# jeffchy/RE2NN-SEQ

Measured on AMD Instinct MI355X. Metric: tagged tokens/sec @ batch=256, seqlen=64; achieved HBM GB/s vs peak, higher is better.
Workload: dtype f32; 1 GPU; ATIS-BIO-sized onehot i-FST (--method onehot --independent 2): V=950 S=71 C=128, batch 256 x seqlen 64 per GPU, lengths U[5,64]; batches_rotated=4, parallelism=batch-sharded x1 (weights replicated)

## Files before the change

### re2nn-seq_amd/csrc/chain_regs.hip

```cpp
#include <hip/hip_runtime.h>
#include <hip/hip_ext.h>

#include "common.hip.h"
#include "host_util.hip.h"
#include "chain_regs.hip.h"

namespace farnn {

int launch_chain_regs(const RegsParams &p, bool maxsr, bool score, hipStream_t s, hipEvent_t e0, hipEvent_t e1) {
    const int NP = RG_NWC * p.G;
    const bool dest = p.dest && !maxsr;
    const size_t lds = (size_t)regs_lds(p.L, p.SP, NP, p.sp.c16, p.sp.Kc, score, RG_RQ, score && bs_label_map_path(p.sp), dest).total * sizeof(float);
    const dim3 grid(2 * p.B), block(RG_WAVES * 64);
    int rc;
    const bool nlx = p.nl != FARNN_NL_NONE && p.nl != FARNN_NL_RELU;
    const bool lmo = score && bs_label_map_path(p.sp);
#define FARNN_LAUNCH_REGS5(MX, SC, NX, LM, DS)                                                 \
    do {                                                                                       \
        if ((rc = raise_lds_limit(chain_regs_kernel<MX, SC, NX, LM, DS>, lds))) return rc;     \
        if (e0 && e1)                                                                          \
            hipExtLaunchKernelGGL((chain_regs_kernel<MX, SC, NX, LM, DS>), grid, block, (uint32_t)lds, s, e0, e1, 0, p); \
        else                                                                                   \
            chain_regs_kernel<MX, SC, NX, LM, DS><<<grid, block, lds, s>>>(p);                \
    } while (0)
#if defined(FARNN_AB)
#define FARNN_LAUNCH_REGS4(MX, SC, NX, LM) do { if (!MX && dest) FARNN_LAUNCH_REGS5(MX, SC, NX, LM, !MX); else FARNN_LAUNCH_REGS5(MX, SC, NX, LM, false); } while (0)
#else
#define FARNN_LAUNCH_REGS4(MX, SC, NX, LM)                                                     \
    do {                                                                                       \
        if (!MX && dest) FARNN_LAUNCH_REGS5(MX, SC, NX, LM, !MX);                              \
        else if constexpr (MX) FARNN_LAUNCH_REGS5(MX, SC, NX, LM, false);                      \
        else return fail(FARNN_EINVAL, "FARNN_NODEST=1: the source-split compute wavefronts of the sum semiring are compiled into the A/B " \
                                       "build only (FARNN_LIB=.../libfarnn_hip_probes.so, csrc/build.py --probes)%s%s"); \
    } while (0)
#endif
#define FARNN_LAUNCH_REGS3(MX, SC, NX) do { if (SC && lmo) FARNN_LAUNCH_REGS4(MX, SC, NX, SC); else FARNN_LAUNCH_REGS4(MX, SC, NX, false); } while (0)
#define FARNN_LAUNCH_REGS(MX, SC) do { if (nlx) FARNN_LAUNCH_REGS3(MX, SC, true); else FARNN_LAUNCH_REGS3(MX, SC, false); } while (0)
    if (maxsr) { if (score) FARNN_LAUNCH_REGS(true, true); else FARNN_LAUNCH_REGS(true, false); }
    else       { if (score) FARNN_LAUNCH_REGS(false, true); else FARNN_LAUNCH_REGS(false, false); }
#undef FARNN_LAUNCH_REGS
#undef FARNN_LAUNCH_REGS3
#undef FARNN_LAUNCH_REGS4
#undef FARNN_LAUNCH_REGS5
    FARNN_HIP_TRY(hipGetLastError());
    return FARNN_OK;
}

}

#if defined(FARNN_PROBES)
extern "C" int farnn_debug_wg_stamps(long long *out, int n_workgroups) {
    if (!out || n_workgroups < 0 || n_workgroups > farnn::WG_STAMP_MAX) return FARNN_EINVAL;
    if (hipDeviceSynchronize() != hipSuccess) return FARNN_EIO;
    return hipMemcpyFromSymbol(out, HIP_SYMBOL(farnn::g_wg_stamps), sizeof(long long) * 16 * (size_t)n_workgroups) == hipSuccess ? FARNN_OK : FARNN_EIO;
}
#endif
```

### re2nn-seq_amd/csrc/chain_regs.hip.h

```cpp
#pragma once
#include "common.hip.h"
#include "score_params.hip.h"
#include "launch_order.hip.h"
#include "chain_regs_params.hip.h"
#include "beside.hip.h"

#ifndef FARNN_ABLATE
#define FARNN_ABLATE 0
#endif

namespace farnn {

__device__ __forceinline__ void lds_flag_set(int *f, int v) {
    asm volatile("" ::: "memory");
    __hip_atomic_store(f, v, __ATOMIC_RELAXED, __HIP_MEMORY_SCOPE_WORKGROUP);
}
__device__ __forceinline__ int lds_flag_get(const int *f) {
    const int v = __hip_atomic_load(f, __ATOMIC_RELAXED, __HIP_MEMORY_SCOPE_WORKGROUP);
    asm volatile("" ::: "memory");
    return v;
}
template <int PSTR = RG_PART_STRIDE>
__device__ __forceinline__ int regs_flag_newest(const float *fbase, int lane) {
    const int *f = reinterpret_cast<const int *>(fbase) + 4 * (lane < RG_NWC ? lane : 0);
    const int v0 = lds_flag_get(f), v1 = lds_flag_get(f + PSTR);
    return max(v0, v1);
}
template <int PSTR = RG_PART_STRIDE>
__device__ __forceinline__ bool regs_rows_reached(const float *fbase, int lane, int rows) {
    return __ballot(regs_flag_newest<PSTR>(fbase, lane) < rows + 1) == 0ull;
}
template <int PSTR = RG_PART_STRIDE>
__device__ __forceinline__ int regs_rows_done(const float *fbase, int lane) {
    int v = regs_flag_newest<PSTR>(fbase, lane);
#pragma unroll
    for (int off = 1; off < 8; off <<= 1) v = min(v, __shfl_xor(v, off, WAVE));
    return __builtin_amdgcn_readfirstlane(v) - 1;
}

__device__ __forceinline__ float quad_sum(float x) {
    x += __int_as_float(__builtin_amdgcn_update_dpp(0, __float_as_int(x), 0xB1, 0xf, 0xf, true));
    x += __int_as_float(__builtin_amdgcn_update_dpp(0, __float_as_int(x), 0x4E, 0xf, 0xf, true));
    return x;
}
__device__ __forceinline__ float quad_max(float x) {
    x = fmaxf(x, __int_as_float(__builtin_amdgcn_update_dpp(0, __float_as_int(x), 0xB1, 0xf, 0xf, true)));
    x = fmaxf(x, __int_as_float(__builtin_amdgcn_update_dpp(0, __float_as_int(x), 0x4E, 0xf, 0xf, true)));
    return x;
}

}
#include "chain_wide.hip.h"
#include "chain_dest.hip.h"
namespace farnn {

#if defined(FARNN_PROBES)
constexpr int WG_STAMP_MAX = 4096;
__device__ long long g_wg_stamps[16 * WG_STAMP_MAX];
#define FARNN_RG_STAMP(i) do { if (probe && lane == 0) stamps[i] = (long long)__builtin_amdgcn_s_memtime(); } while (0)
#else
#define FARNN_RG_STAMP(i) do { } while (0)
#endif

template <bool MAXSR, bool SCORE, bool NLX, int RQ = RG_RQ, int D = RG_D, bool LMO = false, bool DEST = false>
__device__ __forceinline__ void chain_regs_body(const RegsParams &p, float *smem, const int tid, const int item, int *b_out) {
    constexpr bool WIDE = RQ != RG_RQ;
    static_assert(!DEST || (!WIDE && !MAXSR), "the destination-split form exists for the narrow kernel and the sum semiring");
    constexpr int PSTR = WIDE ? rgw_part_stride(RQ) : RG_PART_STRIDE;
    constexpr int NG = WIDE ? RGW_NG : RG_NG;
    const int lane = tid & 63;
    const int w = __builtin_amdgcn_readfirstlane(tid >> 6);
    constexpr int nthreads = RG_WAVES * 64;
    const int dir = item & 1, slot = item >> 1;
    const int S = p.S, SP = p.SP, G = p.G, RPG = p.RPG, NP = RG_NWC * G;
    const int PS = WIDE ? p.PS : SP;
    const bool lm_path = SCORE && (LMO || bs_label_map_path(p.sp));
    const RegsLds lds = regs_lds(p.L, SP, NP, p.sp.c16, p.sp.Kc, SCORE, RQ, lm_path, DEST);
    long long *tokoff = reinterpret_cast<long long *>(smem + lds.tok);
    float *part = smem + lds.part, *ol = smem + lds.ol, *hist = smem + lds.hist;
    float *ab = smem + lds.ab, *scl = smem + lds.scl, *obuf = smem + lds.obuf;
    int *misc = reinterpret_cast<int *>(smem + lds.misc);

    int b = p.order ? p.order[slot] : slot;
    int len_sel = -1;
    if (p.sort) b = select_by_length_rank(p.len, p.B, p.L, p.pair ? folded_rank(slot, p.B) : slot, reinterpret_cast<int *>(hist), tid, nthreads, &len_sel);
    if (b_out) *b_out = b;
    const int len = len_sel >= 0 ? len_sel : clamp_len(p.len[b], p.L);
    const int nsteps = p.full ? p.L : len;
    const float *hinit = dir == 0 ? p.h0 : p.hT;
#if defined(FARNN_PROBES)
    __shared__ long long stamps[8];
    const bool quiet = (p.dbg & 2048) != 0;
    const bool probe = ((p.dbg & 32768) && nsteps == p.L && p.L >= 32) || quiet;
    if (w == 0) FARNN_RG_STAMP(0);
#endif

    constexpr bool PRIME_EARLY = DEST && (!SCORE || LMO);
    DestRing<RD_D, RD_LPR> dring;
    if constexpr (PRIME_EARLY)
        if (w < RG_NWC && nsteps > 0) regs_dest_prime<RD_D, RD_LPR>(p, dir, w, lane, nsteps, len, b, dring);
    for (int k = tid; k < nsteps; k += nthreads) {
        const int idx = (dir == 0) ? k : (k < len ? len - 1 - k : k);
        tokoff[k] = (long long)clamp_tok(p.x[(long long)b * p.L + idx], p.V) * p.blk * 4;
    }
    for (int j = tid; j < SP; j += nthreads) ol[j] = (p.o && j < S) ? p.o[j] : 1.0f;
    for (int j = tid; j < (nsteps + 1) * SP; j += nthreads) hist[j] = (j < S) ? hinit[j] : 0.0f;
    if (tid < 32) misc[tid] = tid == RGM_ACQ ? -1 : 0;
    if (tid < 2) part[tid * PSTR + PSTR - 1] = MAXSR ? -INFINITY : 0.0f;
    if (tid < 2 * 4 * RG_NWC) {
        const int fb = tid / (4 * RG_NWC), fk = tid % (4 * RG_NWC);
// ... 16 lines not shown
    int kmid = 0, pubmax = 0;
    if (SCORE) bs_halves(dir, len, nsteps, kmid, pubmax);
    BesideParams bs;
    bs.A = p.A; bs.Bk = p.Bk; bs.B = p.B; bs.L = p.L; bs.SP = p.SP; bs.CPR = p.CPR; bs.prog = p.prog; bs.arr = p.arr;
    bs.done = p.done; bs.spin = p.spin; bs.dbg = p.dbg; bs.sp = p.sp;
    bs.epoch = (SCORE && w >= RG_NWC) ? (p.done ? bs_launch_epoch(p.done, lane) : p.epoch_host) : 0u;
    int wr_next = 0;
    unsigned lm_pk0 = 0u, lm_pk1 = 0u;
    if (lm_path) lm_load_packed(bs.sp.lm, lane, lm_pk0, lm_pk1);
    if (w < RG_NWC) {
        if constexpr (WIDE) {
            if (nsteps > 0) {
                __builtin_amdgcn_s_setprio(2);
                regs_compute_wide<MAXSR, NLX, RQ, D>(p, dir, w, lane, nsteps, tokoff, part, ol, hist, smem + lds.xch);
                __builtin_amdgcn_s_setprio(0);
                if (w == 0) FARNN_RG_STAMP(2);
#if defined(FARNN_PROBES)
                if (!SCORE && probe && !quiet && w == 0 && lane == 0)
                    printf("seq %d dir %d (wide): setup %lld, chain %lld (%lld per step)\n", b, dir, stamps[1] - stamps[0], stamps[2] - stamps[1],
                           (stamps[2] - stamps[1]) / nsteps);
#endif
            }
        } else if constexpr (DEST) {
            if (nsteps > 0) {
                __builtin_amdgcn_s_setprio(2);
#if defined(FARNN_PROBES)
                const bool probe_ = probe;
#else
                const bool probe_ = false;
#endif
                if constexpr (!PRIME_EARLY) regs_dest_prime<RD_D, RD_LPR>(p, dir, w, lane, nsteps, len, b, dring);
                regs_compute_dest<NLX, RD_D, RD_LPR>(p, dir, w, lane, nsteps, tokoff, part + NP * PS, ol, hist, smem + lds.xd, probe_, b, dring);
                __builtin_amdgcn_s_setprio(0);
                if (w == 0) FARNN_RG_STAMP(2);
#if defined(FARNN_PROBES)
                if (!SCORE && probe && !quiet && w == 0 && lane == 0)
                    printf("seq %d dir %d (destination split): setup %lld, chain %lld (%lld per step)\n", b, dir, stamps[1] - stamps[0], stamps[2] - stamps[1],
                           (stamps[2] - stamps[1]) / nsteps);
#endif
            }
        } else if (nsteps > 0) {
            __builtin_amdgcn_s_setprio(2);
            int g = lane / p.CPR;
            const int c = lane - g * p.CPR;
            const bool active = g < G;
            if (!active) g = 0;
            const int gid = w * G + g, row0 = gid * RPG;
            unsigned voff[RG_RQ];
#pragma unroll
            for (int u = 0; u < RG_RQ; u++) voff[u] = ((unsigned)(row0 + u) * (unsigned)SP + (unsigned)c * 4u) * 4u;
            const char *Mbase = reinterpret_cast<const char *>(dir == 0 ? p.Mf : p.Mb);
            const int rows_w = G * RPG;
            const int rj = lane >> 2, rs = lane & 3;
            const int my_row = w * rows_w + rj;
            const bool my_valid = rj < rows_w && my_row < S;
            const bool my_writer = my_valid && rs == 0;
            const float my_o = my_valid ? ol[my_row] : 1.0f;
            const float c_pre = dir == 0 ? my_o : 1.0f, c_post = dir == 0 ? 1.0f : my_o;
            const float ninf = -INFINITY;
            bool okrow[RG_RQ];
#pragma unroll
            for (int u = 0; u < RG_RQ; u++) okrow[u] = u < RPG && row0 + u < S;
            constexpr int NQI = (RG_NWC * RG_MAXG + 3) / 4;
            const float *ident = part + RG_PART_STRIDE - 1;
            float *dump = part + 2 * RG_PART_STRIDE;
            const float *qptr[NQI];
// ... 163 lines not shown
                    }
#endif
                    FARNN_RG_PHASE(3);
                }
            }
            if (lane == 0) lds_flag_set(reinterpret_cast<int *>(fslot), nsteps + 1);
#if defined(FARNN_PROBES)
            if (probe && w == 0 && lane == 0 && (p.dbg & 256))
                printf("seq %d dir %d chain phases, cycles per step: block wait %lld, fma + store + issue %lld, partner wait + partial reads %lld, reduce + exchange %lld\n",
                       b, dir, ph[0] / nsteps, ph[1] / nsteps, ph[2] / nsteps, ph[3] / nsteps);
#endif
#undef FARNN_RG_PHASE
#undef FARNN_RG_ISSUE
#undef FARNN_RG_BASE
#undef FARNN_RG_WINDOW
#undef FARNN_RG_WAIT
            __builtin_amdgcn_s_setprio(0);
            if (w == 0) FARNN_RG_STAMP(2);
#if defined(FARNN_PROBES)
            if (!SCORE && probe && !quiet && w == 0 && lane == 0)
                printf("seq %d dir %d: setup %lld, chain %lld (%lld per step)\n", b, dir, stamps[1] - stamps[0], stamps[2] - stamps[1],
                       (stamps[2] - stamps[1]) / nsteps);
#endif
        }
    } else if (w == RG_NWC) {
        if (SCORE && dir == 0) {
            for (int i = nsteps + lane; i < p.L; i += WAVE)
                if (p.sp.tags) p.sp.tags[(long long)b * p.L + i] = -1;
            if (p.sp.scores)
                for (long long e = (long long)nsteps * p.sp.K + lane; e < (long long)p.L * p.sp.K; e += WAVE)
                    p.sp.scores[(long long)b * p.L * p.sp.K + e] = 0.0f;
        }
        int published = -1;
        auto copy_rows = [&](int r0, int r1) {
            const float *src = hist + r0 * SP;
            float *dst = stash + (long long)r0 * SP;
            const int nfl = (r1 - r0 + 1) * SP;
            if (SCORE) {
                for (int j = 2 * lane; j < nfl; j += 2 * WAVE) st2_agent(dst + j, src[j], src[j + 1]);
            } else {
                for (int j = lane; j < nfl; j += WAVE) dst[j] = src[j];
            }
        };
        if (!SCORE && !p.A) wr_next = nsteps + 1;
        while (wr_next <= nsteps) {
            const int done = nsteps > 0 ? regs_rows_done<PSTR>(sflag, lane) : 0;
            if (done < wr_next) { __builtin_amdgcn_s_sleep(1); continue; }
            if (SCORE && nsteps > 0 && wr_next > pubmax && done >= nsteps) break;
            const int hi = min(done, (SCORE && wr_next <= pubmax) ? pubmax : nsteps);
            copy_rows(wr_next, hi);
            wr_next = hi + 1;
            if (SCORE && hi < nsteps && published < pubmax) {
                published = hi;
                asm volatile("s_waitcnt vmcnt(0)" ::: "memory");
                if (lane == 0)
                    __hip_atomic_store(p.prog + (long long)dir * p.B + b, ((unsigned long long)bs.epoch << 32) | (unsigned)published,
                                       __ATOMIC_RELAXED, __HIP_MEMORY_SCOPE_AGENT);
            }
        }
    } else if (SCORE) {
        const int fo = bs_flat_offset(bs, b, lane);
        if (lane == 0) misc[RGM_FOFF] = fo;
        const long long foff = fo;
        unsigned mine = 0u;
        int acq = -1;
        const unsigned long long *oprog = p.prog + (long long)(dir ^ 1) * p.B + b;
        const int kfirst = dir == 0 ? kmid : kmid - 1, kstep = dir == 0 ? 1 : -1, klast = dir == 0 ? ntl : -1;
        if constexpr (!LMO)
        for (int k = kfirst; k != klast && !lm_path; k += kstep) {
            int na, nb;
            bs_tile_need(k, len, nsteps, na, nb);
            const int need_own = dir == 0 ? na : nb, need_oth = dir == 0 ? nb : na;
            if (nsteps - need_own < p.solo_margin) break;
            while (!regs_rows_reached<PSTR>(sflag, lane, need_own)) __builtin_amdgcn_s_sleep(4);
            if (need_oth > acq) {
                int pr = -1;
                for (;;) {
                    pr = lane == 0 ? bs_read_prog(oprog, bs.epoch) : 0;
                    pr = __builtin_amdgcn_readfirstlane(pr);
                    if (pr >= need_oth) break;
                    if (regs_rows_reached<PSTR>(sflag, lane, nsteps)) break;
                    __builtin_amdgcn_s_sleep(8);
                }
                if (pr < need_oth) break;
                __builtin_amdgcn_fence(__ATOMIC_ACQUIRE, "agent");
                acq = pr;
            }
            {
                const rg_f32x4 none[NG] = {};
                bs_score_tiles<false, RG_WAVES, NG, RG_NWC>(bs, b, dir, len, nsteps, k, -1, hist, nullptr, nullptr, ab, scl, foff, 0, lane, none);
            }
            mine |= 1u << k;
        }
        {
            int slot = 0;
            for (int k = kfirst; k != klast && slot < RG_NOB; k += kstep) {
                if ((mine >> k) & 1u) continue;
                int na, nb;
                bs_tile_need(k, len, nsteps, na, nb);
                const int need_oth = dir == 0 ? nb : na;
                if (need_oth > acq) {
                    int pr = -1;
                    for (;;) {
                        pr = lane == 0 ? bs_read_prog(oprog, bs.epoch) : 0;
                        pr = __builtin_amdgcn_readfirstlane(pr);
                        if (pr >= need_oth) break;
                        if (regs_rows_reached<PSTR>(sflag, lane, nsteps)) break;
                        __builtin_amdgcn_s_sleep(16);
                    }
                    if (pr < need_oth) break;
                    __builtin_amdgcn_fence(__ATOMIC_ACQUIRE, "agent");
                    acq = pr;
                }
                bs_park_rows<NG, (LMO && WIDE) ? NG / 2 : NG>(bs, b, dir, len, nsteps, k, obuf + slot * RG_TT * SP, lane);
                if (lane == 0) misc[RGM_PARK + slot] = k + 1;
                slot++;
            }
        }
        if (lane == 0) { misc[RGM_MINE] = (int)mine; misc[RGM_ACQ] = acq; }
        FARNN_RG_STAMP(3);
    }
    if constexpr (!SCORE) {
        if (b_out && dir == 0 && w == RG_WAVES - 1) {
            int partsum = 0;
            if (p.sp.flat && !p.sp.offs)
                for (int j = lane; j < b; j += WAVE) partsum += clamp_len(p.len[j], p.L);
#pragma unroll
            for (int off = 32; off >= 1; off >>= 1) partsum += __shfl_xor(partsum, off, WAVE);
            if (lane == 0) { misc[RGM_FOFF] = partsum; misc[RGM_FOFF + 1] = len; }
        }
        return;
    }

    if (w == 0) FARNN_RG_STAMP(4);
    bs_finish<RG_WAVES, NG, RG_WAVES - 1, RG_NWC, true, LMO>(bs, b, dir, len, nsteps, kmid, hist, ab, scl, obuf, misc, w, lane, lm_pk0, lm_pk1, bs.epoch,
        [&]() {
            if (w == RG_NWC)
                for (; wr_next <= nsteps; wr_next++)
                    for (int j = 2 * lane; j < SP; j += 2 * WAVE)
                        st2_agent(stash + (long long)wr_next * SP + j, hist[wr_next * SP + j], hist[wr_next * SP + j + 1]);
        },
        [&]() {
            if (w == RG_NWC) {
                asm volatile("s_waitcnt vmcnt(0)" ::: "memory");
                if (lane == 0)
                    __hip_atomic_store(p.prog + (long long)dir * p.B + b, ((unsigned long long)bs.epoch << 32) | (unsigned)nsteps,
                                       __ATOMIC_RELAXED, __HIP_MEMORY_SCOPE_AGENT);
            }
        });
#if defined(FARNN_PROBES)
    if (quiet && tid == 0 && item < WG_STAMP_MAX) {
        long long *o = g_wg_stamps + 16 * (long long)item + 8;
        o[0] = stamps[1] - stamps[0]; o[1] = stamps[2] - stamps[1]; o[2] = stamps[3] - stamps[2]; o[3] = stamps[4] - stamps[2];
        o[4] = (long long)__builtin_amdgcn_s_memtime() - stamps[4];
    }
    if (probe && !quiet && tid == 0) {
        const long long e = (long long)__builtin_amdgcn_s_memtime();
        printf("seq %d dir %d: setup %lld, chain %lld (%lld per step), scorer alone until +%lld, all waves at the meeting point +%lld, "
               "tiles + arrival %lld; tiles alone %d of %d\n", b, dir, stamps[1] - stamps[0], stamps[2] - stamps[1],
               (stamps[2] - stamps[1]) / nsteps, stamps[3] - stamps[2], stamps[4] - stamps[2], e - stamps[4],
               __popc((unsigned)misc[RGM_MINE]), ntl);
    }
#endif
}

template <bool MAXSR, bool SCORE, bool NLX, bool LMO = false, bool DEST = false>
__global__ void __launch_bounds__(RG_WAVES * 64, 4)
chain_regs_kernel(const RegsParams p) {
    extern __shared__ __align__(16) float smem[];
#if defined(FARNN_PROBES)
    long long w0r = 0, w0c = 0;
    if ((p.dbg & 2048) && threadIdx.x == 0) { w0r = (long long)__builtin_amdgcn_s_memrealtime(); w0c = (long long)__builtin_amdgcn_s_memtime(); }
    int b_probe = -1;
    chain_regs_body<MAXSR, SCORE, NLX, RG_RQ, RG_D, LMO, DEST>(p, smem, (int)threadIdx.x, (int)blockIdx.x, &b_probe);
    if ((p.dbg & 2048) && threadIdx.x == 0 && blockIdx.x < WG_STAMP_MAX) {
        const long long w1r = (long long)__builtin_amdgcn_s_memrealtime(), w1c = (long long)__builtin_amdgcn_s_memtime();
        unsigned hwid, xcc;
        asm volatile("s_getreg_b32 %0, hwreg(HW_REG_HW_ID)" : "=s"(hwid));
        asm volatile("s_getreg_b32 %0, hwreg(HW_REG_XCC_ID)" : "=s"(xcc));
        long long *o = g_wg_stamps + 16 * (long long)blockIdx.x;
        o[0] = b_probe; o[1] = b_probe >= 0 ? (long long)p.len[b_probe] : -1; o[2] = w0r; o[3] = w1r; o[4] = w1c - w0c;
        o[5] = xcc & 15u; o[6] = (hwid >> 13) & 7u; o[7] = (hwid >> 8) & 15u;
    }
#else
    chain_regs_body<MAXSR, SCORE, NLX, RG_RQ, RG_D, LMO, DEST>(p, smem, (int)threadIdx.x, (int)blockIdx.x, nullptr);
#endif
}

template <bool MAXSR, bool SCORE, bool NLX, int RQ, int D>
__global__ void __launch_bounds__(RG_WAVES * 64, 2)
chain_wide_kernel(const RegsParams p) {
    extern __shared__ __align__(16) float smem[];
    chain_regs_body<MAXSR, SCORE, NLX, RQ, D>(p, smem, (int)threadIdx.x, (int)blockIdx.x, nullptr);
}

template <bool MAXSR, bool NLX, int RQ>
__global__ void __launch_bounds__(RG_WAVES * 64, 4)
chain_wide_paired_kernel(const RegsParams p) {
    extern __shared__ __align__(16) float smem[];
    chain_regs_body<MAXSR, true, NLX, RQ, 2, true>(p, smem, (int)threadIdx.x, (int)blockIdx.x, nullptr);
}

}
```

### re2nn-seq_amd/csrc/chain_regs_params.hip.h

```cpp
#pragma once
#include <hip/hip_runtime.h>
#include "common.hip.h"
#include "score_params.hip.h"

namespace farnn {

constexpr int RG_NWC = 6;
constexpr int RG_WAVES = 8;
constexpr int RG_D = 4;
constexpr int RG_RQ = 4;
constexpr int RG_MAXG = 4;
constexpr int RG_MAXSP = 72;
constexpr int RG_PART_STRIDE = RG_NWC * RG_MAXG * RG_MAXSP;
constexpr int RGW_G = 2;
constexpr int RGW_NP = RG_NWC * RGW_G;
constexpr int RGW_MAXSP = 128;
constexpr int RGW_MAXRQ = 11;
__host__ __device__ constexpr int rgw_part_stride(int rq) { return rq <= 9 ? 1536 : 2048; }
constexpr int RGW_XCH = 32;
constexpr int RD_LPR = 5;
constexpr int RD_XS = 80;
constexpr int RD_D = 4;
constexpr int RD_XD_FLOATS = 2 * RD_XS + 128;

// ... 28 lines not shown
    int G, RPG, NP, CPR, SP, rows;
    bool ok;
    bool wide;
    int RQ, D, PS;
};

inline RegsGeom regs_geometry(int S) {
    RegsGeom g;
    g.wide = false; g.RQ = RG_RQ; g.D = RG_D; g.PS = 0;
    g.SP = round_up(S, 4);
    g.CPR = g.SP / 4;
    g.ok = g.CPR <= 64 && S >= 1;
    g.G = g.ok ? 64 / g.CPR : 1;
    if (g.G > RG_MAXG) g.G = RG_MAXG;
    g.NP = RG_NWC * g.G;
    g.RPG = (S + g.NP - 1) / g.NP;
    if (g.RPG > RG_RQ) g.ok = false;
    g.rows = (g.NP - 1) * g.RPG + RG_RQ;
    if (g.NP * g.SP + 4 * RG_NWC + 4 * (64 - g.G * g.CPR) >= RG_PART_STRIDE) g.ok = false;
    if (!g.ok && S > 4 * RG_RQ && g.SP <= RGW_MAXSP) {
        g.wide = true;
        g.G = RGW_G; g.NP = RGW_NP;
        g.RPG = (S + g.NP - 1) / g.NP;
        g.RQ = g.RPG <= 8 ? 8 : (g.RPG <= 9 ? 9 : RGW_MAXRQ);
        g.D = 4;
        g.rows = g.NP * g.RPG;
        g.PS = ((g.SP + 15) & ~31) + 16;
        g.ok = g.RPG <= RGW_MAXRQ && g.NP * g.PS + 4 * RG_NWC + 4 * (64 - g.G * g.CPR) < rgw_part_stride(g.RQ);
    }
    return g;
}

struct RegsLds {
    int tok, hp, part, ol, hist, ab, scl, obuf, misc, xch, xd, total;
};
__host__ __device__ inline RegsLds regs_lds(int L, int SP, int NP, int c16, int Kc, bool score, int rq = RG_RQ, bool lm = false, bool dest = false) {
    const bool wide = rq != RG_RQ;
    RegsLds l;
    int at = 0;
    l.tok = at;  at += 2 * ((L + 1) & ~1);
    l.hp = at;
    l.part = at; at += 2 * (wide ? rgw_part_stride(rq) : RG_PART_STRIDE) + 64 * 4;
    l.ol = at;   at += SP;
    l.hist = at; at += (L + 1) * SP + 16;
    l.ab = at;   at += (score && !lm) ? 2 * RG_TT * (16 * c16 + 4) : 0;
    l.scl = at;  at += (score && !lm) ? 2 * RG_TT * Kc : 0;
    l.obuf = at; at += score ? 2 * RG_TT * SP : 0;
    l.misc = at; at += 32;
    l.xch = at;  at += wide ? RG_NWC * RGW_XCH : 0;
    l.xd = at;   at += dest ? RD_XD_FLOATS : 0;
    l.total = at;
    return l;
}

int launch_chain_regs(const RegsParams &p, bool maxsr, bool score, hipStream_t s, hipEvent_t e0, hipEvent_t e1);
int launch_chain_wide(const RegsParams &p, bool maxsr, bool score, hipStream_t s, hipEvent_t e0, hipEvent_t e1);
int launch_chain_wide_paired(const RegsParams &p, bool maxsr, hipStream_t s, hipEvent_t e0, hipEvent_t e1);

bool chain_viterbi_fits(int L, int SP, int NP, int K, int Kp, bool label_map, int rq = RG_RQ);
int launch_chain_viterbi(const RegsParams &p, const ScoreParams &sp, bool maxsr, hipStream_t s, hipEvent_t e0, hipEvent_t e1);

}
```

### re2nn-seq_amd/csrc/farnn_hip.hip

```cpp
#include <hip/hip_runtime.h>
#include <hip/hip_ext.h>
#include <stdlib.h>
#include <algorithm>
#include <map>
#include <new>
#include <utility>
#include <vector>

#include "common.hip.h"
#include "host_util.hip.h"
#include "chain.hip.h"
#include "score_decode.hip.h"
#include "layout.hip.h"
#include "fst4_score.hip.h"
#include "decomp_chain.hip.h"
#include "decomp1_score.hip.h"
#include "decomp_rows.hip.h"
#include "compact_tag.hip.h"
#include "decomp_regs.hip.h"
#include "compact.hip.h"
#include "host_util.hip.h"
#include "chain_regs_params.hip.h"

namespace farnn {
// ... 35 lines not shown
    float *o = nullptr, *h0 = nullptr, *hT = nullptr;
    float *OT = nullptr, *P = nullptr, *tr = nullptr;
    float *OTm = nullptr; int c16 = 0;
    LabelMap lm = {nullptr, 0, 0, -1, 0.0f, 0, 0, 0.0f};
    DecompWeights dw;
    DecompRowsPack rows;
    int RO = 0, ROp = 0;
    float *d1_S1o = nullptr, *d1_S2o = nullptr, *d1_CoutT = nullptr;
    float *d1_BSSp = nullptr;
    float *d1_S1oP = nullptr;
    float *d1_S2oP = nullptr;
    int n_cu = 0;
    int RW = 0, RWp = 0;
    float *d0_Vgen = nullptr, *d0_CT = nullptr, *d0_S1w = nullptr, *d0_S2w = nullptr, *d0_CwT = nullptr;
    float *A = nullptr, *Bk = nullptr, *crf_scores = nullptr;
    float *d1_br = nullptr;
    int64_t *offs = nullptr;
    int *order = nullptr;
    int wsB = 0, wsL = 0;
    int curL = 0;
    ChainGeom geom;
    RegsGeom rgeom;
    unsigned long long *hs = nullptr;
    size_t hs_bytes = 0;
    unsigned epoch_u = 0;
    bool last_regs = false;
    bool last_lm_score = false;
    int chain_ks = 3;
    bool prep_in_kernel = false, sort_in_kernel = false;
    bool dense_decomp = false;
    bool order_valid = false;
    bool last_wave = false;
    bool last_fused = false;
    int profiling = 0;
    long long calls = 0;
    int prof_this_call = 0;
    Prof prof;
    std::vector<void *> owned;
    struct HostSlot {
        int64_t *x_pin = nullptr, *flat_pin = nullptr;
        int64_t *x_dev = nullptr, *flat_dev = nullptr, *x_map = nullptr;
        size_t capN = 0, capB = 0;
        long long total = 0;
        hipEvent_t ev_out = nullptr;
        bool busy = false;
        unsigned gen = 0;
    } hslot[FARNN_HOST_SLOTS];
    hipStream_t hs_run = nullptr;
    int hnext = 0;
    hipStream_t last_stream = nullptr;
    bool have_last = false, multi_stream = false;
    hipEvent_t ev_order = nullptr;
};

static int dev_alloc(farnn_model *m, void **p, size_t bytes) {
    FARNN_HIP_TRY(hipMalloc(p, bytes + 1024));
    m->owned.push_back(*p);
    return FARNN_OK;
}

static int dev_upload(farnn_model *m, float **dst, const float *src, size_t n, size_t n_alloc,
                      int on_device) {
    int rc = dev_alloc(m, (void **)dst, n_alloc * sizeof(float));
    if (rc) return rc;
    FARNN_HIP_TRY(hipMemset(*dst, 0, n_alloc * sizeof(float)));
    if (src && n)
// ... 350 lines not shown

extern "C" int farnn_set_profiling(farnn_model *m, int32_t enable) {
    if (!m) return fail(FARNN_EINVAL, "null model%s%s");
    prof_fold(m);
    if (enable) {
        for (int k = 0; k < KERN_COUNT; k++) { m->prof.ms[k] = 0; m->prof.n[k] = 0; }
        while (m->prof.pool.size() < 256) {
            hipEvent_t e = nullptr;
            if (hipEventCreate(&e) != hipSuccess) break;
            m->prof.pool.push_back(e);
        }
    }
    m->profiling = enable > 0 ? enable : 0;
    m->calls = 0;
    return FARNN_OK;
}

extern "C" int farnn_kernel_time(farnn_model *m, int32_t which, double *total_ms, int64_t *launches) {
    if (!m || which < 0 || which >= KERN_COUNT) return fail(FARNN_EINVAL, "kernel_time: bad arguments%s%s");
    prof_fold(m);
    if (total_ms) *total_ms = m->prof.ms[which];
    if (launches) *launches = m->prof.n[which];
    return FARNN_OK;
}

extern "C" const char *farnn_kernel_name(const farnn_model *m, int32_t which) {
    if (!m) return "";
    TunScope tun_scope(&m->tun);
    switch (which) {
        case KERN_CHAIN:
            if (m->compact_on) return m->last_fused ? "compact_tag_kernel<fused: both chains + label-map scores + decode>" : "compact_chain_kernel";
            if (m->last_regs && m->last_fused && m->use_crf) return "chain_viterbi_kernel<fused: recurrence + scores + CRF decode>";
            if (m->last_regs && m->rgeom.wide) return m->last_fused ? "chain_wide_kernel<fused: scores + decode beside the recurrence>" : "chain_wide_kernel";
            if (m->last_regs) return m->last_fused ? "chain_regs_kernel<fused: scores + decode beside the recurrence>" : "chain_regs_kernel";
            if (m->dense_decomp) return "chain_kernel";
            if (m->kind == KIND_DECOMP && m->last_fused && m->last_wave) return "decomp_regs_kernel<fused: scores + decode beside the recurrence>";
            if (m->kind == KIND_DECOMP || m->kind == KIND_DECOMP1 || m->kind == KIND_DECOMP0)
                return m->rows.ok ? ((m->last_wave || (m->calls == 0 && m->dw.farnn == 0 && m->dw.R <= DG_ROWS && !tun(TUN_DECOMP_NOREGS))) ? "decomp_regs_kernel" : "decomp_rows_kernel") : "decomp_chain_kernel";
            return "chain_kernel";
        case KERN_SCORE: return m->kind == KIND_FST4 ? "fst4_score_kernel"
                              : (m->kind == KIND_IND1 ? "ind1_score_kernel"
                              : (m->kind == KIND_DECOMP1 ? (m->d1_BSSp ? "decomp1_br_mfma_kernel+decomp1_label_kernel" : "decomp1_score_kernel")
                              : (m->kind == KIND_DECOMP0 ? "decomp0_score_kernel"
                              : (m->use_crf ? "score_tile_kernel+viterbi_kernel" : (m->last_lm_score ? "label_map_score_kernel" : "score_tile_kernel")))));
        case KERN_PREP:  return "batch_prep_kernel";
        default: return "";
    }
}


static RegsParams make_regs_params(farnn_model *m, const int64_t *x, const int64_t *len, int B, int full) {
    const RegsGeom &rg = m->rgeom;
    RegsParams rp;
    memset(&rp, 0, sizeof(rp));
    rp.Mf = m->Mf; rp.Mb = m->Mb; rp.blk = (long long)m->geom.SR * m->SP;
    rp.o = m->o; rp.h0 = m->h0; rp.hT = m->hT; rp.x = x; rp.len = len;
    rp.order = m->order_valid ? m->order : nullptr; rp.sort = m->sort_in_kernel ? 1 : 0;
    rp.A = m->A; rp.Bk = m->Bk; rp.B = B; rp.L = m->curL; rp.S = m->S; rp.SP = m->SP; rp.CPR = rg.CPR; rp.V = m->V;
    rp.G = rg.G; rp.RPG = rg.RPG; rp.RQ = rg.RQ; rp.D = rg.D; rp.PS = rg.PS; rp.pair = rg.wide ? 0 : 1;
    rp.nl = m->nl; rp.full = full; rp.dbg = tun(TUN_DBG);
    rp.dest = (!rg.wide && m->semiring != FARNN_SEMIRING_MAX && !tun(TUN_NODEST)) ? 1 : 0;
    return rp;
}

static int handoff_words(farnn_model *m, unsigned long long **prog, unsigned long long **arr, unsigned long long **done) {
    *prog = m->hs; *arr = m->hs + (size_t)2 * m->wsB; *done = m->hs + (size_t)3 * m->wsB + 16;
    return FARNN_OK;
}

static int launch_chain(farnn_model *m, const int64_t *x, const int64_t *len, int B, int L, int full,
                        hipStream_t s, const ScoreParams *fuse_sp = nullptr, bool *fused = nullptr) {
    const ChainGeom &g = m->geom;
    if (fused) *fused = false;
    m->last_regs = false;
    if (m->rgeom.ok && !tun(TUN_NOREGS)) {
        const RegsGeom &rg = m->rgeom;
        const size_t lds_cap = rg.wide ? 158 * 1024 : 80 * 1024;
        bool score = fuse_sp && m->hs && m->OTm && m->c16 >= 1 && m->c16 <= (rg.wide ? RGW_NG : RG_NG) && m->Kc <= 256 && m->curL <= 31 * RG_TT &&
                     (B <= 1024 || !fuse_sp->flat || fuse_sp->offs) && !tun(TUN_NOFUSE);
        if (score && !rg.wide && bs_label_map_path(*fuse_sp) && !tun(TUN_FUSE)) score = false;
        const bool lm_path = score && bs_label_map_path(*fuse_sp);
        const bool dest = !rg.wide && m->semiring != FARNN_SEMIRING_MAX && !tun(TUN_NODEST);
        size_t lds = (size_t)regs_lds(m->curL, m->SP, rg.NP, score ? m->c16 : 0, score ? m->Kc : 0, score, rg.RQ, lm_path, dest).total * sizeof(float);
        const bool paired = rg.wide && lm_path && rg.RQ <= 9 && lds <= 80 * 1024 && !tun(TUN_WIDE_UNPAIRED);
        if (score && lds > lds_cap) {
            score = false;
            lds = (size_t)regs_lds(m->curL, m->SP, rg.NP, 0, 0, false, rg.RQ, false, dest).total * sizeof(float);
        }
        if (lds <= lds_cap) {
            RegsParams rp = make_regs_params(m, x, len, B, full);
            if (score) {
                int hrc = handoff_words(m, &rp.prog, &rp.arr, &rp.done);
                if (hrc) return hrc;
                if (tun(TUN_HOST_EPOCH)) {
                    if (++m->epoch_u == 0) { FARNN_HIP_TRY(hipMemsetAsync(m->hs, 0, m->hs_bytes, s)); m->epoch_u = 1; }
                    rp.done = nullptr; rp.epoch_host = m->epoch_u + 0x40000000u;
                }
                rp.spin = tun(TUN_FUSE_SPIN);
                rp.solo_margin = tun(TUN_SOLO_MARGIN);
                rp.sp = *fuse_sp;
                if (fused) *fused = true;
            }
            KernelTimer kt(m, KERN_CHAIN, s, true);
            if (paired && score) { rp.D = 2; rp.pair = 1; }
            const int rc = (paired && score) ? launch_chain_wide_paired(rp, m->semiring == FARNN_SEMIRING_MAX, s, kt.e0, kt.e1)
                           : rg.wide ? launch_chain_wide(rp, m->semiring == FARNN_SEMIRING_MAX, score, s, kt.e0, kt.e1)
                                     : launch_chain_regs(rp, m->semiring == FARNN_SEMIRING_MAX, score, s, kt.e0, kt.e1);
            if (rc) return rc;
            m->last_regs = true;
            return FARNN_OK;
        }
    }
    (void)fuse_sp;
    ChainParams p;
    p.Mf = m->Mf; p.Mb = m->Mb; p.blk = (long long)m->geom.SR * m->SP;
    p.o = m->o; p.h0 = m->h0; p.hT = m->hT; p.x = x; p.len = len; p.A = m->A; p.Bk = m->Bk;
    p.order = m->order_valid ? m->order : nullptr;
    p.sort = m->sort_in_kernel ? 1 : 0;
    p.B = B; p.L = m->curL; p.S = m->S; p.SP = m->SP; p.CPR = g.CPR; p.V = m->V;
    p.NW = g.NW; p.NLD = g.NLD; p.G = g.G; p.LPR = g.LPR; p.RPG = g.RPG; p.RPGp = g.RPGp; p.NQ = g.NQ;
    p.nl = m->nl; p.full = full; p.dbg = tun(TUN_DBG);
    int ks = 2, nqp = g.NQ;
    if (!g.pick_ring(m->curL, m->chain_ks, ks, nqp))
        return fail(FARNN_ERANGE, "chain kernel: LDS ring does not fit (sequence too long for this S)%s%s");
    p.KS = ks; p.NQP = nqp; p.PPS = (g.NQ + nqp - 1) / nqp;
    const size_t lds = g.lds_bytes(m->curL, ks, nqp);
    dim3 grid(2 * B), block((g.NW + g.NLD + 1) * 64);
    const bool mx = m->semiring == FARNN_SEMIRING_MAX;
    int rc = FARNN_OK;
    if (tun(TUN_CHAIN_HELPER) && block.x < 512) block = dim3(block.x + 64);
#define FARNN_LAUNCH_CHAIN(NCH, MX, FQ)                                                       \
    do {                                                                                      \
        if ((rc = raise_lds_limit(chain_kernel<NCH, MX, FQ>, lds))) return rc;                \
        if (kt.e0 && kt.e1)                                                                   \
            hipExtLaunchKernelGGL((chain_kernel<NCH, MX, FQ>), grid, block, (uint32_t)lds, s, kt.e0, kt.e1, 0, p); \
        else                                                                                  \
            chain_kernel<NCH, MX, FQ><<<grid, block, lds, s>>>(p);                            \
    } while (0)
#define FARNN_LAUNCH_CHAIN_MX(NCH, FQ)                                                        \
    do { if (mx) FARNN_LAUNCH_CHAIN(NCH, true, FQ); else FARNN_LAUNCH_CHAIN(NCH, false, FQ); } while (0)
    KernelTimer kt(m, KERN_CHAIN, s, true);
    const int fq_max = block.x <= 384 ? 6 : 3;
// ... 1348 lines not shown
```

Before: 301.6 million tokens/s.

## Fuse label-map tagging into the chain kernel via a later-chain epilogue

Adds a TAIL variant of the destination-split recurrence kernel. Each direction publishes its history rows, and the second chain of a sequence to arrive, detected through an atomic exchange on a per-sequence arrival word, computes the label-map scores and writes the tags directly. This removes the separate scoring/decode kernel launch and its reread of the state histories. In exchange it adds agent-scope atomics and fences and a serial epilogue on whichever workgroup finishes last.

```diff
diff --git a/re2nn-seq_amd/csrc/chain_regs.hip b/re2nn-seq_amd/csrc/chain_regs.hip
--- a/re2nn-seq_amd/csrc/chain_regs.hip
+++ b/re2nn-seq_amd/csrc/chain_regs.hip
@@ -7,10 +7,12 @@
 
 namespace farnn {
 
-int launch_chain_regs(const RegsParams &p, bool maxsr, bool score, hipStream_t s, hipEvent_t e0, hipEvent_t e1) {
+int launch_chain_regs(const RegsParams &p, bool maxsr, bool score, hipStream_t s, hipEvent_t e0, hipEvent_t e1, bool tail) {
     const int NP = RG_NWC * p.G;
     const bool dest = p.dest && !maxsr;
-    const size_t lds = (size_t)regs_lds(p.L, p.SP, NP, p.sp.c16, p.sp.Kc, score, RG_RQ, score && bs_label_map_path(p.sp), dest).total * sizeof(float);
+    if (tail && (!dest || score || !p.arr || !p.done))
+        return fail(FARNN_EINVAL, "chain_regs: the tagging epilogue belongs to the recurrence-only destination-split kernel%s%s");
+    const size_t lds = (size_t)regs_lds(p.L, p.SP, NP, p.sp.c16, p.sp.Kc, score, RG_RQ, score && bs_label_map_path(p.sp), dest, tail).total * sizeof(float);
     const dim3 grid(2 * p.B), block(RG_WAVES * 64);
     int rc;
     const bool nlx = p.nl != FARNN_NL_NONE && p.nl != FARNN_NL_RELU;
@@ -36,12 +38,23 @@
 #endif
 #define FARNN_LAUNCH_REGS3(MX, SC, NX) do { if (SC && lmo) FARNN_LAUNCH_REGS4(MX, SC, NX, SC); else FARNN_LAUNCH_REGS4(MX, SC, NX, false); } while (0)
 #define FARNN_LAUNCH_REGS(MX, SC) do { if (nlx) FARNN_LAUNCH_REGS3(MX, SC, true); else FARNN_LAUNCH_REGS3(MX, SC, false); } while (0)
+#define FARNN_LAUNCH_REGS6(NX)                                                                 \
+    do {                                                                                       \
+        if ((rc = raise_lds_limit(chain_regs_kernel<false, false, NX, false, true, true>, lds))) return rc; \
+        if (e0 && e1)                                                                          \
+            hipExtLaunchKernelGGL((chain_regs_kernel<false, false, NX, false, true, true>), grid, block, (uint32_t)lds, s, e0, e1, 0, p); \
+        else                                                                                   \
+            chain_regs_kernel<false, false, NX, false, true, true><<<grid, block, lds, s>>>(p); \
+    } while (0)
+    if (tail) { if (nlx) FARNN_LAUNCH_REGS6(true); else FARNN_LAUNCH_REGS6(false); }
+    else
     if (maxsr) { if (score) FARNN_LAUNCH_REGS(true, true); else FARNN_LAUNCH_REGS(true, false); }
     else       { if (score) FARNN_LAUNCH_REGS(false, true); else FARNN_LAUNCH_REGS(false, false); }
 #undef FARNN_LAUNCH_REGS
 #undef FARNN_LAUNCH_REGS3
 #undef FARNN_LAUNCH_REGS4
 #undef FARNN_LAUNCH_REGS5
+#undef FARNN_LAUNCH_REGS6
     FARNN_HIP_TRY(hipGetLastError());
     return FARNN_OK;
 }
diff --git a/re2nn-seq_amd/csrc/chain_regs.hip.h b/re2nn-seq_amd/csrc/chain_regs.hip.h
--- a/re2nn-seq_amd/csrc/chain_regs.hip.h
+++ b/re2nn-seq_amd/csrc/chain_regs.hip.h
@@ -4,6 +4,7 @@
 #include "launch_order.hip.h"
 #include "chain_regs_params.hip.h"
 #include "beside.hip.h"
+#include "chain_tail.hip.h"
 
 #ifndef FARNN_ABLATE
 #define FARNN_ABLATE 0
@@ -62,10 +63,11 @@
 #define FARNN_RG_STAMP(i) do { } while (0)
 #endif
 
-template <bool MAXSR, bool SCORE, bool NLX, int RQ = RG_RQ, int D = RG_D, bool LMO = false, bool DEST = false>
+template <bool MAXSR, bool SCORE, bool NLX, int RQ = RG_RQ, int D = RG_D, bool LMO = false, bool DEST = false, bool TAIL = false>
 __device__ __forceinline__ void chain_regs_body(const RegsParams &p, float *smem, const int tid, const int item, int *b_out) {
     constexpr bool WIDE = RQ != RG_RQ;
     static_assert(!DEST || (!WIDE && !MAXSR), "the destination-split form exists for the narrow kernel and the sum semiring");
+    static_assert(!TAIL || (DEST && !SCORE && !LMO), "the tail is the epilogue of the recurrence-only destination-split kernel");
     constexpr int PSTR = WIDE ? rgw_part_stride(RQ) : RG_PART_STRIDE;
     constexpr int NG = WIDE ? RGW_NG : RG_NG;
     const int lane = tid & 63;
@@ -75,7 +77,7 @@
     const int S = p.S, SP = p.SP, G = p.G, RPG = p.RPG, NP = RG_NWC * G;
     const int PS = WIDE ? p.PS : SP;
     const bool lm_path = SCORE && (LMO || bs_label_map_path(p.sp));
-    const RegsLds lds = regs_lds(p.L, SP, NP, p.sp.c16, p.sp.Kc, SCORE, RQ, lm_path, DEST);
+    const RegsLds lds = regs_lds(p.L, SP, NP, p.sp.c16, p.sp.Kc, SCORE, RQ, lm_path, DEST, TAIL);
     long long *tokoff = reinterpret_cast<long long *>(smem + lds.tok);
     float *part = smem + lds.part, *ol = smem + lds.ol, *hist = smem + lds.hist;
     float *ab = smem + lds.ab, *scl = smem + lds.scl, *obuf = smem + lds.obuf;
@@ -158,6 +160,7 @@
                 if constexpr (!PRIME_EARLY) regs_dest_prime<RD_D, RD_LPR>(p, dir, w, lane, nsteps, len, b, dring);
                 regs_compute_dest<NLX, RD_D, RD_LPR>(p, dir, w, lane, nsteps, tokoff, part + NP * PS, ol, hist, smem + lds.xd, probe_, b, dring);
                 __builtin_amdgcn_s_setprio(0);
+                if constexpr (TAIL) asm volatile("s_waitcnt vmcnt(0)" ::: "memory");
                 if (w == 0) FARNN_RG_STAMP(2);
 #if defined(FARNN_PROBES)
                 if (!SCORE && probe && !quiet && w == 0 && lane == 0)
@@ -387,11 +390,13 @@
                     p.sp.scores[(long long)b * p.L * p.sp.K + e] = 0.0f;
         }
         int published = -1;
+        unsigned tail_epoch = 0u;
+        if constexpr (TAIL) tail_epoch = bs_launch_epoch(p.done, lane);
         auto copy_rows = [&](int r0, int r1) {
             const float *src = hist + r0 * SP;
             float *dst = stash + (long long)r0 * SP;
             const int nfl = (r1 - r0 + 1) * SP;
-            if (SCORE) {
+            if (SCORE || TAIL) {
                 for (int j = 2 * lane; j < nfl; j += 2 * WAVE) st2_agent(dst + j, src[j], src[j + 1]);
             } else {
                 for (int j = lane; j < nfl; j += WAVE) dst[j] = src[j];
@@ -413,6 +418,17 @@
                                        __ATOMIC_RELAXED, __HIP_MEMORY_SCOPE_AGENT);
             }
         }
+        if constexpr (TAIL) {
+            const bool second = tail_arrive(p.arr, p.done, tail_epoch, b, p.B, lane);
+            if (lane == 0) misc[RGM_TODO] = second ? 1 : 0;
+        }
+    } else if (TAIL) {
+        const int fo = bs_flat_offset(bs, b, lane);
+        if (lane == 0) misc[RGM_FOFF] = fo;
+        unsigned pk0, pk1;
+        lm_load_packed(p.sp.lm, lane, pk0, pk1);
+        unsigned *lmt = reinterpret_cast<unsigned *>(smem + lds.lmt);
+        lmt[lane] = pk0; lmt[64 + lane] = pk1;
     } else if (SCORE) {
         const int fo = bs_flat_offset(bs, b, lane);
         if (lane == 0) misc[RGM_FOFF] = fo;
@@ -475,6 +491,12 @@
         if (lane == 0) { misc[RGM_MINE] = (int)mine; misc[RGM_ACQ] = acq; }
         FARNN_RG_STAMP(3);
     }
+    if constexpr (TAIL) {
+        wg_barrier_lds();
+        if (misc[RGM_TODO])
+            tail_tag_sequence<RG_WAVES>(p.sp, b, dir, len, nsteps, hist, reinterpret_cast<const unsigned *>(smem + lds.lmt), (long long)misc[RGM_FOFF], w, lane);
+        return;
+    }
     if constexpr (!SCORE) {
         if (b_out && dir == 0 && w == RG_WAVES - 1) {
             int partsum = 0;
@@ -519,7 +541,7 @@
 #endif
 }
 
-template <bool MAXSR, bool SCORE, bool NLX, bool LMO = false, bool DEST = false>
+template <bool MAXSR, bool SCORE, bool NLX, bool LMO = false, bool DEST = false, bool TAIL = false>
 __global__ void __launch_bounds__(RG_WAVES * 64, 4)
 chain_regs_kernel(const RegsParams p) {
     extern __shared__ __align__(16) float smem[];
@@ -527,7 +549,7 @@
     long long w0r = 0, w0c = 0;
     if ((p.dbg & 2048) && threadIdx.x == 0) { w0r = (long long)__builtin_amdgcn_s_memrealtime(); w0c = (long long)__builtin_amdgcn_s_memtime(); }
     int b_probe = -1;
-    chain_regs_body<MAXSR, SCORE, NLX, RG_RQ, RG_D, LMO, DEST>(p, smem, (int)threadIdx.x, (int)blockIdx.x, &b_probe);
+    chain_regs_body<MAXSR, SCORE, NLX, RG_RQ, RG_D, LMO, DEST, TAIL>(p, smem, (int)threadIdx.x, (int)blockIdx.x, &b_probe);
     if ((p.dbg & 2048) && threadIdx.x == 0 && blockIdx.x < WG_STAMP_MAX) {
         const long long w1r = (long long)__builtin_amdgcn_s_memrealtime(), w1c = (long long)__builtin_amdgcn_s_memtime();
         unsigned hwid, xcc;
@@ -538,7 +560,7 @@
         o[5] = xcc & 15u; o[6] = (hwid >> 13) & 7u; o[7] = (hwid >> 8) & 15u;
     }
 #else
-    chain_regs_body<MAXSR, SCORE, NLX, RG_RQ, RG_D, LMO, DEST>(p, smem, (int)threadIdx.x, (int)blockIdx.x, nullptr);
+    chain_regs_body<MAXSR, SCORE, NLX, RG_RQ, RG_D, LMO, DEST, TAIL>(p, smem, (int)threadIdx.x, (int)blockIdx.x, nullptr);
 #endif
 }
 
diff --git a/re2nn-seq_amd/csrc/chain_regs_params.hip.h b/re2nn-seq_amd/csrc/chain_regs_params.hip.h
--- a/re2nn-seq_amd/csrc/chain_regs_params.hip.h
+++ b/re2nn-seq_amd/csrc/chain_regs_params.hip.h
@@ -84,9 +84,10 @@
 }
 
 struct RegsLds {
-    int tok, hp, part, ol, hist, ab, scl, obuf, misc, xch, xd, total;
+    int tok, hp, part, ol, hist, ab, scl, obuf, misc, xch, xd, lmt, total;
 };
-__host__ __device__ inline RegsLds regs_lds(int L, int SP, int NP, int c16, int Kc, bool score, int rq = RG_RQ, bool lm = false, bool dest = false) {
+__host__ __device__ inline RegsLds regs_lds(int L, int SP, int NP, int c16, int Kc, bool score, int rq = RG_RQ, bool lm = false, bool dest = false,
+                                            bool tail = false) {
     const bool wide = rq != RG_RQ;
     RegsLds l;
     int at = 0;
@@ -101,11 +102,12 @@
     l.misc = at; at += 32;
     l.xch = at;  at += wide ? RG_NWC * RGW_XCH : 0;
     l.xd = at;   at += dest ? RD_XD_FLOATS : 0;
+    l.lmt = at;  at += tail ? 2 * 64 : 0;
     l.total = at;
     return l;
 }
 
-int launch_chain_regs(const RegsParams &p, bool maxsr, bool score, hipStream_t s, hipEvent_t e0, hipEvent_t e1);
+int launch_chain_regs(const RegsParams &p, bool maxsr, bool score, hipStream_t s, hipEvent_t e0, hipEvent_t e1, bool tail = false);
 int launch_chain_wide(const RegsParams &p, bool maxsr, bool score, hipStream_t s, hipEvent_t e0, hipEvent_t e1);
 int launch_chain_wide_paired(const RegsParams &p, bool maxsr, hipStream_t s, hipEvent_t e0, hipEvent_t e1);
 
diff --git a/re2nn-seq_amd/csrc/chain_tail.hip.h b/re2nn-seq_amd/csrc/chain_tail.hip.h
--- /dev/null
+++ b/re2nn-seq_amd/csrc/chain_tail.hip.h
@@ -0,0 +1,77 @@
+#pragma once
+#include "common.hip.h"
+#include "score_params.hip.h"
+#include "beside.hip.h"
+
+namespace farnn {
+
+__device__ __forceinline__ bool tail_arrive(unsigned long long *arr, unsigned long long *done, const unsigned epoch, const int b,
+                                            const int B, const int lane) {
+    asm volatile("s_waitcnt vmcnt(0)" ::: "memory");
+    unsigned long long old = 0ull;
+    if (lane == 0)
+        old = __hip_atomic_exchange(arr + b, ((unsigned long long)epoch << 32) | 1ull, __ATOMIC_RELAXED, __HIP_MEMORY_SCOPE_AGENT);
+    const bool second = (unsigned)__builtin_amdgcn_readfirstlane((int)(unsigned)(old >> 32)) == epoch;
+    if (second) {
+        __builtin_amdgcn_fence(__ATOMIC_ACQUIRE, "agent");
+        asm volatile("s_waitcnt vmcnt(0)" ::: "memory");
+        if (lane == 0) __hip_atomic_fetch_add(done, bs_epoch_add(b, B), __ATOMIC_RELAXED, __HIP_MEMORY_SCOPE_AGENT);
+    }
+    return second;
+}
+
+template <int NWV>
+__device__ __forceinline__ void tail_tag_sequence(const ScoreParams &sp, const int b, const int dir, const int len, const int nsteps,
+                                                  const float *hist, const unsigned *lmt, const long long foff, const int w,
+                                                  const int lane) {
+    const int L = sp.L, SP = sp.SP;
+    if (sp.tags)
+#pragma clang loop vectorize(disable) unroll(disable)
+        for (int i = nsteps + w * WAVE + lane; i < L; i += NWV * WAVE) sp.tags[(long long)b * L + i] = -1;
+    if (2 * w >= nsteps) return;
+    LabelMapRegs lr;
+    lm_unpack(sp.lm, lmt[lane], lmt[64 + lane], lr);
+    const bool two = sp.lm.nq > 1;
+    const bool fwd = dir == 0;
+    const float *oth = (fwd ? sp.Bk : sp.A) + (long long)b * (L + 1) * SP;
+    auto rowB = [&](int i) { return (i + 1 <= len) ? len - (i + 1) : i + 1; };
+    auto own_row = [&](int i) { return fwd ? i + 1 : rowB(i); };
+    auto oth_row = [&](int i) { return fwd ? rowB(i) : i + 1; };
+    float oa0 = 0.f, oa1 = 0.f, ob0 = 0.f, ob1 = 0.f;
+    auto fetch = [&](int q) {
+        const int ia = q, ib = q + 1 < nsteps ? q + 1 : q;
+        const float *ra = oth + (long long)oth_row(ia) * SP, *rb = oth + (long long)oth_row(ib) * SP;
+        oa0 = __hip_atomic_load(ra + lr.st0, __ATOMIC_RELAXED, __HIP_MEMORY_SCOPE_AGENT);
+        ob0 = __hip_atomic_load(rb + lr.st0, __ATOMIC_RELAXED, __HIP_MEMORY_SCOPE_AGENT);
+        if (two) {
+            oa1 = __hip_atomic_load(ra + lr.st1, __ATOMIC_RELAXED, __HIP_MEMORY_SCOPE_AGENT);
+            ob1 = __hip_atomic_load(rb + lr.st1, __ATOMIC_RELAXED, __HIP_MEMORY_SCOPE_AGENT);
+        }
+    };
+    int q = 2 * w;
+    fetch(q);
+    for (; q < nsteps; q += 2 * NWV) {
+        const bool hasb = q + 1 < nsteps;
+        const int ia = q, ib = hasb ? q + 1 : q;
+        const float *ha = hist + own_row(ia) * SP, *hb = hist + own_row(ib) * SP;
+        const float wa0 = ha[lr.st0], wb0 = hb[lr.st0];
+        const float wa1 = two ? ha[lr.st1] : 0.0f, wb1 = two ? hb[lr.st1] : 0.0f;
+        const float xa0 = (fwd ? wa0 : oa0) * (fwd ? oa0 : wa0), xb0 = (fwd ? wb0 : ob0) * (fwd ? ob0 : wb0);
+        const float xa1 = two ? (fwd ? wa1 : oa1) * (fwd ? oa1 : wa1) : 0.0f, xb1 = two ? (fwd ? wb1 : ob1) * (fwd ? ob1 : wb1) : 0.0f;
+        if (q + 2 * NWV < nsteps) fetch(q + 2 * NWV);
+        float ya0, ya1, yb0, yb1;
+        lm_scan_scores2(lr, xa0, xa1, xb0, xb1, ya0, ya1, yb0, yb1);
+        float ma = fmaxf(ya0, ya1), mb = fmaxf(yb0, yb1);
+        wave_max_dpp2(ma, mb);
+        const int taga = lm_tag_from_candidates(sp.lm, lr, ya0, ya1, ma, sp.K, sp.o_idx);
+        const int tagb = lm_tag_from_candidates(sp.lm, lr, yb0, yb1, mb, sp.K, sp.o_idx);
+        if (lane < (hasb ? 2 : 1)) {
+            const int i = lane ? ib : ia;
+            const int tag = lane ? tagb : taga;
+            if (sp.tags) sp.tags[(long long)b * L + i] = tag;
+            if (sp.flat && i < len) sp.flat[foff + i] = tag;
+        }
+    }
+}
+
+}
diff --git a/re2nn-seq_amd/csrc/farnn_hip.hip b/re2nn-seq_amd/csrc/farnn_hip.hip
--- a/re2nn-seq_amd/csrc/farnn_hip.hip
+++ b/re2nn-seq_amd/csrc/farnn_hip.hip
@@ -91,6 +91,7 @@
     bool order_valid = false;
     bool last_wave = false;
     bool last_fused = false;
+    bool last_tail = false;
     int profiling = 0;
     long long calls = 0;
     int prof_this_call = 0;
@@ -507,6 +508,7 @@
             if (m->compact_on) return m->last_fused ? "compact_tag_kernel<fused: both chains + label-map scores + decode>" : "compact_chain_kernel";
             if (m->last_regs && m->last_fused && m->use_crf) return "chain_viterbi_kernel<fused: recurrence + scores + CRF decode>";
             if (m->last_regs && m->rgeom.wide) return m->last_fused ? "chain_wide_kernel<fused: scores + decode beside the recurrence>" : "chain_wide_kernel";
+            if (m->last_regs && m->last_tail) return "chain_regs_kernel<tags by the later chain>";
             if (m->last_regs) return m->last_fused ? "chain_regs_kernel<fused: scores + decode beside the recurrence>" : "chain_regs_kernel";
             if (m->dense_decomp) return "chain_kernel";
             if (m->kind == KIND_DECOMP && m->last_fused && m->last_wave) return "decomp_regs_kernel<fused: scores + decode beside the recurrence>";
@@ -543,11 +545,17 @@
     return FARNN_OK;
 }
 
+static bool tail_form_wins(int B, int L, int S) {
+    (void)B; (void)L; (void)S;
+    return true;
+}
+
 static int launch_chain(farnn_model *m, const int64_t *x, const int64_t *len, int B, int L, int full,
                         hipStream_t s, const ScoreParams *fuse_sp = nullptr, bool *fused = nullptr) {
     const ChainGeom &g = m->geom;
     if (fused) *fused = false;
     m->last_regs = false;
+    m->last_tail = false;
     if (m->rgeom.ok && !tun(TUN_NOREGS)) {
         const RegsGeom &rg = m->rgeom;
         const size_t lds_cap = rg.wide ? 158 * 1024 : 80 * 1024;
@@ -556,7 +564,9 @@
         if (score && !rg.wide && bs_label_map_path(*fuse_sp) && !tun(TUN_FUSE)) score = false;
         const bool lm_path = score && bs_label_map_path(*fuse_sp);
         const bool dest = !rg.wide && m->semiring != FARNN_SEMIRING_MAX && !tun(TUN_NODEST);
-        size_t lds = (size_t)regs_lds(m->curL, m->SP, rg.NP, score ? m->c16 : 0, score ? m->Kc : 0, score, rg.RQ, lm_path, dest).total * sizeof(float);
+        const bool tail = fuse_sp && !score && dest && m->hs && bs_label_map_path(*fuse_sp) && (B <= 1024 || !fuse_sp->flat || fuse_sp->offs) &&
+                          !tun(TUN_NOFUSE) && !tun(TUN_FUSE) && tail_form_wins(B, m->curL, m->S);
+        size_t lds = (size_t)regs_lds(m->curL, m->SP, rg.NP, score ? m->c16 : 0, score ? m->Kc : 0, score, rg.RQ, lm_path, dest, tail).total * sizeof(float);
         const bool paired = rg.wide && lm_path && rg.RQ <= 9 && lds <= 80 * 1024 && !tun(TUN_WIDE_UNPAIRED);
         if (score && lds > lds_cap) {
             score = false;
@@ -576,13 +586,20 @@
                 rp.sp = *fuse_sp;
                 if (fused) *fused = true;
             }
+            if (tail) {
+                int hrc = handoff_words(m, &rp.prog, &rp.arr, &rp.done);
+                if (hrc) return hrc;
+                rp.sp = *fuse_sp;
+                if (fused) *fused = true;
+            }
             KernelTimer kt(m, KERN_CHAIN, s, true);
             if (paired && score) { rp.D = 2; rp.pair = 1; }
             const int rc = (paired && score) ? launch_chain_wide_paired(rp, m->semiring == FARNN_SEMIRING_MAX, s, kt.e0, kt.e1)
                            : rg.wide ? launch_chain_wide(rp, m->semiring == FARNN_SEMIRING_MAX, score, s, kt.e0, kt.e1)
-                                     : launch_chain_regs(rp, m->semiring == FARNN_SEMIRING_MAX, score, s, kt.e0, kt.e1);
+                                     : launch_chain_regs(rp, m->semiring == FARNN_SEMIRING_MAX, score, s, kt.e0, kt.e1, tail);
             if (rc) return rc;
             m->last_regs = true;
+            m->last_tail = tail;
             return FARNN_OK;
         }
     }
```

Result: slower. 297.8 million tokens/s (-1.3%).
